# jonathan-innis/karpenter-provider-aws

Hardware: AMD Instinct MI355X
Metric: pods scheduled/sec (Solve, 50k pods × EC2 catalog) (higher is better)
Workload: dtype int64; 1 GPU; config2: 50000 heterogeneous pods (250 classes) x 918 types x 3 AZ x {spot,on-demand}, 2 NodePools; pods=50000, types=918, parallelism=single

## Files before the change

karpenter-provider-aws_amd/csrc/kp_ffd.h:

```cpp
#pragma once
#include <hip/hip_runtime.h>
#include <stdint.h>

#include <type_traits>

#include "kp_bound.h"
#include "kp_device.h"
#include "kp_eval.h"
#include "kp_gosort.h"
#include "kp_layout.h"

namespace KP_WNS {

#ifdef KP_NO_TOPO
#define KP_TOPO_ON 0
#else
#define KP_TOPO_ON 1
#endif

__device__ __forceinline__ bool ports_meet(const KpDev& d, const uint64_t* m, int c) {
    uint64_t x = 0;
    for (int w = 0; w < d.PW; w++)
        x |= __hip_atomic_load(const_cast<uint64_t*>(m) + w, __ATOMIC_RELAXED, __HIP_MEMORY_SCOPE_AGENT) &
             d.cls_ports[(size_t)c * d.PW + w];
// ... 318 lines not shown
        for (uint64_t m = ballot(live); m; m &= m - 1) {
            const int j = __ffsll((unsigned long long)m) - 1;
            const int g = rl32(R.g, j), flags = rl32(R.flags, j), key = rl32(R.key, j);
            if (flags & 8) {
                if (lane == 0) {
                    const int old = atomicAdd(&d.tg_hcnt[(size_t)(-1 - key) * d.HN + d.E + nc], 1);
                    if (old == 0) atomicAdd(&d.tg_pos[g], 1);
                }
                continue;
            }
            const uint64_t wv = rl64(w, j);
            if ((wv >> lane) & 1ull) atomicAdd(&d.tg_cnt[(size_t)g * 64 + lane], 1);
            if (lane == 0 && wv) atomicOr((unsigned long long*)&d.tg_known[g], (unsigned long long)wv);
        }
    }
    if (keep && lane == 0) {
        S.tr_n = nr;
        S.tr_cls = c;
    }
    asm volatile("s_waitcnt vmcnt(0)" ::: "memory");
}

#define KP_CAND_VIRT 0x40000000
#ifndef KP_BOUND_SWEEP
#define KP_BOUND_SWEEP 0
#endif
#ifndef KP_BOUND_IDLE_WAVE
#define KP_BOUND_IDLE_WAVE 1
#endif
#ifndef KP_BOUND_ROW_SKIP
#define KP_BOUND_ROW_SKIP 1
#endif
#ifndef KP_BOUND_TMPL_IDLE
#define KP_BOUND_TMPL_IDLE 1
#endif
template <bool PROF>
static __device__ __attribute__((noinline)) int bound_round(const int64_t* __restrict__ nc_bound,
                                                            const int64_t* __restrict__ nc_req,
                                                            int R, int A,
                                                            FfdShared& S, uint32_t* key, const uint16_t* ord, int buf,
                                                            int cnt, int sdone, int r) {
    static_assert(KP_NWAVES <= 8 && KP_LDS_AXES <= KP_BOUND_STRIDE && KP_BOUND_STRIDE == 8, "lane = 8 candidate + axis");
    const int lane = (int)__lane_id(), ci = lane >> 3, ai = lane & 7;
    const bool v = ci < cnt && ai < A;
    const int nc = ord[S.cand_pos[buf][ci < cnt ? ci : 0]];
    const int64_t b = v ? __hip_atomic_load(const_cast<int64_t*>(&nc_bound[(size_t)nc * KP_BOUND_STRIDE + ai]), __ATOMIC_RELAXED,
                                            __HIP_MEMORY_SCOPE_AGENT) : KP_NO_BOUND;
    const int64_t tot = v ? ld_req(&nc_req[(size_t)nc * R + r]) : 0;
    const uint64_t m = ballot(v && kp_bound_rejects(b, tot, S.pod_req[r]));
    if (!m) return 0;
    uint64_t vm = 0;
    for (int i = 0; i < 8; i++)
        if ((m >> (8 * i)) & 0xFFull) vm |= 1ull << i;
    const int nv = __popcll(vm);
    const int p = lane < cnt ? S.cand_pos[buf][lane] : 0;
    const bool rej = (vm >> lane) & 1ull;
    if (nv == cnt && !sdone) {
        if (rej) key[p] |= 0x80000000u;
        if (lane == 0) {
            S.st[ST_NC_EVALS] += cnt;
            S.st[ST_BOUND_SKIPS] += cnt;
            if (PROF) S.st[ST_BOUND_ALLV]++;
            S.fwd = 1;
        }
        return 1;
    }
    if (rej) S.cand_pos[buf][lane] = p | KP_CAND_VIRT;
    if (PROF && lane == 0) S.st[nv == cnt ? ST_BOUND_ALLV : ST_BOUND_MIXED]++;
    return 0;
}
template <bool TOPO, bool PORTS = false, bool BOUND = false, bool PROF = false>
__device__ inline bool collect_candidates(const KpDev& d, FfdShared& S,
                                          std::conditional_t<PORTS || BOUND, uint32_t*, const uint32_t*> key,
                                          const uint16_t* ord, const uint8_t* stmpl, uint64_t tol, int N, int start, int buf,
                                          int lane, int pc = -1, bool bound = false) {
    int pos = start;
    bool marked = false;
    for (;;) {
        int cnt = 0, next = N;
        const int tp_n = TOPO ? S.tp_n : 0;
        const int L = tp_n ? d.topo_cands : KP_NWAVES;
        while (pos < N) {
            const int p = pos + lane;
            bool c = p < N && !(key[p] >> 31);
            if (c) c = (tol >> stmpl[ord[p]]) & 1ull;
            if (PORTS && pc >= 0) {
                const bool meet = c && ports_meet(d, d.nc_ports + (size_t)ord[p] * d.PW, pc);
                if constexpr (PORTS)
                    if (meet) key[p] |= 0x80000000u;
                marked |= ballot(meet) != 0;
                c = c && !meet;
            }
            if (tp_n && c) c = topo_prefilter_pass(d, S, ord[p]);
            const uint64_t m0 = __ballot(c);
            if (tp_n && m0 && cnt + __popcll(m0) < L) {
                const int rank = cnt + __popcll(m0 & ((1ull << lane) - 1ull));
                if (c) S.cand_pos[buf][rank] = p;
                cnt += __popcll(m0);
                pos += 64;
                if (lane == 0) {
                    S.n_cand[buf] = cnt;
                    S.scan_next[buf] = pos < N ? pos : N;
// ... 98 lines not shown
        if (!pending || base >= TP) break;
#pragma unroll
        for (int ai = 0; ai < KP_LDS_AXES; ai++) t[ai] = ((pending >> ai) & 1u) ? (int)rank[ai * TP + base + lane] : 0xFFFF;
    }
#endif
    tail.hi = (tail.hi & 0x0000FFFFFFFFFFFFull) | ((uint64_t)(unsigned)(first < 0 ? start : first) << 48);
    int64_t mine = KP_NO_BOUND;
#pragma unroll
    for (int ai = 0; ai < KP_LDS_AXES; ai++)
        if (lane == ai) mine = mx[ai];
    if (lane < A)
        __hip_atomic_store(&row[lane], kp_bound_entry(mine, ws.hr[lane] >= 0), __ATOMIC_RELAXED, __HIP_MEMORY_SCOPE_AGENT);
    if (lane == KP_BOUND_STRIDE - 2 || lane == KP_BOUND_STRIDE - 1)
        __hip_atomic_store(&row[lane], (int64_t)(lane == KP_BOUND_STRIDE - 2 ? tail.lo : tail.hi), __ATOMIC_RELAXED,
                           __HIP_MEMORY_SCOPE_AGENT);
}

__device__ __forceinline__ uint64_t limit_filter(const KpDev& d, int j, uint64_t o, int lane) {
    return lane < d.TW ? o & d.tmpl_lmask[(size_t)j * d.TW + lane] : o;
}

__device__ inline void limit_mask_update(const KpDev& d, int j, int lane) {
    uint32_t lm = 0;
    for (int r = 0; r < d.R; r++)
        if (d.limit_set[(size_t)j * d.R + r]) lm |= 1u << r;
    uint64_t mine = ~0ull;
    for (int w = 0; w < d.TW && lm; w++) {
        const int t = w * 64 + lane;
        bool keep = t < d.T;
        for (uint32_t m = lm; m && keep; m &= m - 1) {
            const int r = __ffs(m) - 1;
            keep = d.cap[(size_t)r * d.T + t] <= ld_req(&d.remaining[(size_t)j * d.R + r]);
        }
        const uint64_t nb = ballot(keep);
        if (lane == w) mine = nb;
    }
    if (lane < d.TW) d.tmpl_lmask[(size_t)j * d.TW + lane] = mine;
}

__device__ __forceinline__ long long prof_clock(bool prof) { return prof ? __builtin_amdgcn_s_memtime() : 0; }


__device__ __forceinline__ void commit_reservations(const KpDev& d, int32_t* rcap, const WaveScratch& ws, int nc,
                                                    bool fresh, int* rel_flag, int lane) {
    const int RW = d.ro_ridw;
    if (lane < RW) {
        uint64_t* hp = d.nc_held + (size_t)nc * RW + lane;
        const uint64_t old = fresh ? 0ull : ld_u64(hp), nh = ws.minbits[lane];
        for (uint64_t x = nh & ~old; x; x &= x - 1) rcap[lane * 64 + __ffsll((unsigned long long)x) - 1]--;
        for (uint64_t x = old & ~nh; x; x &= x - 1)
            if (rcap[lane * 64 + __ffsll((unsigned long long)x) - 1]++ == 0) *rel_flag = 1;
        __hip_atomic_store(hp, nh, __ATOMIC_RELAXED, __HIP_MEMORY_SCOPE_AGENT);
    }
    if (lane == 0) __hip_atomic_store(&d.nc_rlive[nc], ws.rlive, __ATOMIC_RELAXED, __HIP_MEMORY_SCOPE_AGENT);
}
__device__ __forceinline__ uint64_t held_word(const KpDev& d, int nc, int lane) {
    return lane < d.ro_ridw ? ld_u64(&d.nc_held[(size_t)nc * d.ro_ridw + lane]) : 0ull;
}

template <bool VOL = false>
// ... 284 lines not shown
        for (int j = 0; j < d.NT; j++)
            if (d.min_keys[(size_t)j * KP_MAX_CLASS_KEYS] >= 0) mmask |= 1ull << j;
        E.min_tmpl_mask = mmask;
    }
    SortSlice sl{skey, sord};
    int my_axis = 0, my_shift = 0;
#pragma unroll
    for (int ai = 0; ai < KP_LDS_AXES; ai++)
        if (lane == ai) {
            my_axis = d.active_axes[ai];
            my_shift = d.qshift[ai];
        }
    const long long pop_bound = (long long)P * 64 + 4096;
    constexpr bool LEAN = !PORTS || TOPO;
    int qw_n = 0, qw_used = 0;
    int vp = 0, vc = 0, vshape = 0, vlast = 0;
    uint64_t vtol = 0;
    int32_t vq[KP_LDS_AXES];
#pragma unroll
    for (int ai = 0; ai < KP_LDS_AXES; ai++) vq[ai] = 0;

    for (;;) {
        const long long c_top = (prof && tid == 0) ? __builtin_amdgcn_s_memtime() : 0;
        if (wave == 0) {
            const long long c_in = prof_clock(prof);
            const int N = S.N;
            int qhead = S.qhead, qcount = S.qcount;
            int seq = S.seq, prev_shape = S.prev_shape, dkind = S.dirty_kind, dpos = S.dirty_pos;
            int sstart = S.scan_start;
            int eager = S.eager;
            int any_rej = S.any_rej;
            const int ep = S.epoch;
            if (PREF && d.relax_next && S.relaxed) {
                vlast = -1;
                __builtin_amdgcn_fence(__ATOMIC_SEQ_CST, "wavefront");
                if (lane == 0) S.relaxed = 0;
            }
            if (RESV && S.rel_flag) {
                for (int i = lane; i < N; i += 64) skey[i] &= KEYMASK;
                any_rej = 0;
                sstart = 0;
                __builtin_amdgcn_fence(__ATOMIC_SEQ_CST, "wavefront");
                if (lane == 0) S.rel_flag = 0;
            }
            int xstart = S.xstart;
            long long nexist = 0;
// ... 566 lines not shown
                            qcount--;
                            popped++;
                            scanned += N;
                            n_inner++;
                            stay = true;
                            break;
                        }
                        t_d = prof_clock(prof);
                        cqinner += t_d - t_e;
                        if (!stay) break;
                        again = false;
                        continue;
                    }
                }
                break;
                }
                if (again) continue;
                t_f = prof_clock(prof);
                ho_fail = t_f - t_d;
                if (prof) {
                    const bool fa = f < N && rl32(wa ? 1 : 0, (f - wb) & 63) != 0;
                    if (lane == 0) S.st[ST_SLOW_WHY + (f >= N ? 0 : A == 0 ? 3 : !fa ? 1 : 2)]++;
                }
                win_flush();
                wb = -1;
                if (lane < R) S.pod_req[lane] = qw_req[off * R + lane];
                if (lane == 0) {
                    S.cur_pod = p;
                    S.cls_fill = S.CC.cls != c;
                    S.topo_pod = 0;
                }
                if (BOUND) asm volatile("s_waitcnt vmcnt(0)" ::: "memory");
                if (BOUND && lane == 0) S.fwd = 0;
                if (collect_candidates<TOPO_ON, PORTS, BOUND, PROF>(d, S, skey, sord, stmpl, ~0ull, N, f, 0, lane,
                                                                          (PORTS && cport) ? c : -1, BOUND))
                    any_rej = 1;
                break;
            }
            win_flush();
            ex_flush();
            const long long t_w = prof_clock(prof);
            if (lane == 0) {
                S.xstart = xstart;
                S.st[ST_EXIST_PLACED] += nexist;
                S.qhead = qhead;
                S.qcount = qcount;
                S.seq = seq;
                S.prev_shape = prev_shape;
                S.dirty_kind = dkind;
                S.dirty_pos = dpos;
                S.scan_start = sstart;
                S.eager = eager;
                S.any_rej = any_rej;
                S.topo_resume = 0;
                S.rej_volatile = 0;
                S.done = done;
// ... 224 lines not shown
                    if (!ok && S.ws[0].memo_ok) {
                        skey[S.cand_pos[b][i]] |= 0x80000000u;
                        S.any_rej = 1;
                    }
                    if (!ok && !S.ws[0].memo_ok) S.rej_volatile = 1;
                    S.st[ST_NC_EVALS]++;
                }
                if (ok) {
                    win = i;
                    break;
                }
            }
            if (win >= 0 || S.scan_done[b]) break;
            if (wave == 0 &&
                collect_candidates<TOPO_ON, PORTS>(d, S, skey, sord, stmpl, S.topo_pod ? d.tol[S.cur_cls] : ~0ull, S.N, S.scan_next[b],
                                                   b ^ 1, lane, (PORTS && (S.CC.flags & CF_PORTS)) ? S.cur_cls : -1) && lane == 0)
                S.any_rej = 1;
            __syncthreads();
            round++;
        }
        int first = 0;
        bool team_won = false;
        if ((KP_TEAM_FIRST_RESV | !RESV) && (KP_TEAM_FIRST_TOPO | !TOPO))
        if (!team && d.team_first && S.n_cand[0] > 0 && !(BOUND && ((S.cand_pos[0][0] & KP_CAND_VIRT) || S.fwd))) {
            const int nc = sord[S.cand_pos[0][0]];
            const int tm = d.nc_tmpl[nc];
            const bool fast0 = !(S.CC.flags & CF_TOPO) && !(RESV && d.resv_on && ld_i32(&d.nc_rlive[nc])) &&
                               (slast[nc] == (uint16_t)S.cur_cls || ((S.CC.flags & CF_NOKEYS) && ((S.CC.tol >> tm) & 1ull)));
            if (!fast0) {
                EvalIn a;
                a.Ahdr = d.nc_hdr + (size_t)nc * K;
                a.Aw = d.nc_words + (size_t)nc * d.DW;
                a.opts = lane < TW ? d.nc_opts[(size_t)nc * TW + lane] : 0;
                a.base_req = d.nc_req + (size_t)nc * R;
                a.pod_req = S.pod_req;
                a.tmpl = tm;
                a.compat = true;
                a.force_off = false;
                a.prof = wave == 0 ? &S.st[ST_EV_REQ] : nullptr;
                a.host = d.E + nc;
                a.held = (RESV && d.resv_on) ? held_word(d, nc, lane) : 0ull;
                TeamBuf* const tb = &S.team[tjoins & 1];
                const bool ok = (TOPO_ON && (S.CC.flags & CF_TOPO_CONS))
                                    ? eval_wave<true, RESV, true, PREF, false, true, PROF>(d, E, S.CC, a, S.ws[wave], lane, tb,
                                                                                     wave, KP_NWAVES, &tjoins)
                                    : eval_wave<false, RESV, true, PREF, false, true, PROF>(d, E, S.CC, a, S.ws[wave], lane,
                                                                                      tb, wave, KP_NWAVES, &tjoins);
                if (wave == 0 && lane == 0) {
                    S.fastp[0][0] = 0;
                    S.acc[0][0] = ok;
                    if (!ok && S.ws[0].memo_ok) {
                        skey[S.cand_pos[0][0]] |= 0x80000000u;
                        S.any_rej = 1;
                    }
                    if (!ok && !S.ws[0].memo_ok) S.rej_volatile = 1;
                    S.st[ST_NC_EVALS]++;
                    if (prof) S.st[ST_SLOW_WHY + 8]++;
                }
                first = 1;
                if (ok) {
                    win = 0;
                    team_won = true;
                }
                __syncthreads();
            }
        }
        for (; !team && !team_won;) {
            const int b = round & 1;
            const int f0 = round == 0 ? first : 0;
            const int ci = wave + f0;
            if (BOUND && ci < S.n_cand[b] && (S.cand_pos[b][ci] & KP_CAND_VIRT)) {
                if (lane == 0) {
                    S.fastp[b][ci] = 0;
                    S.acc[b][ci] = 0;
                    skey[S.cand_pos[b][ci] & ~KP_CAND_VIRT] |= 0x80000000u;
                    S.any_rej = 1;
                    atomicAdd((unsigned long long*)&S.st[ST_BOUND_SKIPS], 1ull);
                }
            } else if (ci < S.n_cand[b]) {
                const int nc = sord[S.cand_pos[b][ci]];
                EvalIn a;
                a.Ahdr = d.nc_hdr + (size_t)nc * K;
                a.Aw = d.nc_words + (size_t)nc * d.DW;
                a.opts = lane < TW ? d.nc_opts[(size_t)nc * TW + lane] : 0;
                a.base_req = d.nc_req + (size_t)nc * R;
// ... 115 lines not shown
            auto commit_tmpl = [&](int jj, int cw) {
                const int n = S.N;
                for (int k = lane; k < K; k += 64) d.nc_hdr[(size_t)n * K + k] = d.cls_hdr[(size_t)(d.C + jj) * K + k];
                for (int i = lane; i < d.DW; i += 64)
                    d.nc_words[(size_t)n * d.DW + i] = d.cls_words[(size_t)(d.C + jj) * d.DW + i];
                asm volatile("s_waitcnt vmcnt(0)" ::: "memory");
                commit_reqs(d, S.CC, S.ws[cw], n, lane);
                if (PREF && d.best_effort) {
                    asm volatile("s_waitcnt vmcnt(0)" ::: "memory");
                    commit_min_relax(d, S.ws[cw], n, lane);
                }
                if (RESV && d.resv_on) commit_reservations(d, sRcap, S.ws[cw], n, true, &S.rel_flag, lane);
                if (TOPO_ON && (S.CC.flags & CF_TOPO))
                    topo_record(d, S.CC, S.ws[cw], d.cls_hdr + (size_t)(d.C + jj) * K,
                                d.cls_words + (size_t)(d.C + jj) * d.DW, d.E + n, jj, true, lane, -1, nullptr,
                                S.born);
                if (lane < TW) d.nc_opts[(size_t)n * TW + lane] = S.ws[cw].opts[lane];
                if (PORTS) nodeclaim_ports_commit(d, n, S.cur_cls, true, jj, lane);
                for (int r = lane; r < R; r += 64)
                    __hip_atomic_store(&d.nc_req[(size_t)n * R + r], d.daemon[(size_t)jj * R + r] + S.pod_req[r],
                                       __ATOMIC_RELAXED, __HIP_MEMORY_SCOPE_AGENT);
                if (lane < A && n < NQ) shr[lane * NQ + n] = S.ws[cw].hr[lane];
                if (BOUND && !KP_BOUND_TMPL_IDLE) bound_row_store<PROF>(d.self, E.alloc, S.ws[cw], n, 0, S.st);
                for (int r = 0; r < R; r++) {
                    if (!d.limit_set[(size_t)jj * R + r]) continue;
                    int64_t mx = INT64_MIN;
                    for (int w2 = 0; w2 < TW; w2++) {
                        const uint64_t ow = S.ws[cw].opts[w2];
                        if ((ow >> lane) & 1ull) {
                            const int64_t cp = d.cap[(size_t)r * T + w2 * 64 + lane];
                            mx = cp > mx ? cp : mx;
                        }
                    }
                    mx = wave_max64(mx);
                    if (lane == 0) d.remaining[(size_t)jj * R + r] -= mx;
                }
                asm volatile("s_waitcnt vmcnt(0)" ::: "memory");
                limit_mask_update(d, jj, lane);
                if (lane == 0) {
                    slast[n] = (uint16_t)S.cur_cls;
                    stmpl[n] = (uint8_t)jj;
                    d.nc_tmpl[n] = jj;
                    sord[n] = (uint16_t)n;
                    skey[n] = 1;
                    S.N = n + 1;
                    S.dirty_kind = 2;
                    S.dirty_pos = n;
                    d.pod_result[pod] = n;
                    d.pod_order[pod] = S.seq++;
                }
                asm volatile("s_waitcnt vmcnt(0)" ::: "memory");
            };
            int twin = -1;
            if (KP_TEAM_TMPL && (!RESV || KP_TEAM_TMPL_RESV) && !TOPO && d.team_first) {
                const int n_new = BOUND ? S.N : 0;
                for (int j = 0; j < d.NT; j++) {
                    uint64_t o = (lane < TW && d.tmpl_ok[j]) ? d.tmpl_opts[(size_t)j * TW + lane] : 0;
                    o = limit_filter(d, j, o, lane);
                    if (PORTS && (S.CC.flags & CF_PORTS) && ports_meet(d, d.tmpl_ports + (size_t)j * d.PW, S.cur_cls)) o = 0;
                    if (!ballot(o != 0)) continue;
                    EvalIn a;
// ... 93 lines not shown
                        const int n = S.N;
                        for (int k = lane; k < K; k += 64) d.nc_hdr[(size_t)n * K + k] = d.cls_hdr[(size_t)(d.C + jj) * K + k];
                        for (int i = lane; i < d.DW; i += 64)
                            d.nc_words[(size_t)n * d.DW + i] = d.cls_words[(size_t)(d.C + jj) * d.DW + i];
                        asm volatile("s_waitcnt vmcnt(0)" ::: "memory");
                        commit_reqs(d, S.CC, S.ws[wave], n, lane);
                        if (PREF && d.best_effort) {
                            asm volatile("s_waitcnt vmcnt(0)" ::: "memory");
                            commit_min_relax(d, S.ws[wave], n, lane);
                        }
                        if (RESV && d.resv_on) commit_reservations(d, sRcap, S.ws[wave], n, true, &S.rel_flag, lane);
                        if (TOPO_ON && (S.CC.flags & CF_TOPO))
                            topo_record(d, S.CC, S.ws[wave], d.cls_hdr + (size_t)(d.C + jj) * K,
                                        d.cls_words + (size_t)(d.C + jj) * d.DW, d.E + n, jj, true, lane, -1, nullptr,
                                        S.born);
                        if (lane < TW) d.nc_opts[(size_t)n * TW + lane] = S.ws[wave].opts[lane];
                        if (PORTS) nodeclaim_ports_commit(d, n, S.cur_cls, true, jj, lane);
                        for (int r = lane; r < R; r += 64)
                            __hip_atomic_store(&d.nc_req[(size_t)n * R + r], d.daemon[(size_t)jj * R + r] + S.pod_req[r],
                                               __ATOMIC_RELAXED, __HIP_MEMORY_SCOPE_AGENT);
                        if (lane < A && n < NQ) shr[lane * NQ + n] = S.ws[wave].hr[lane];
                        if (BOUND)
                            bound_row_store<PROF>(d.self, E.alloc, S.ws[wave], n, KP_BOUND_TMPL_IDLE ? d.tmpl_bstep[jj] : 0, S.st);
                        for (int r = 0; r < R; r++) {
                            if (!d.limit_set[(size_t)jj * R + r]) continue;
                            int64_t mx = INT64_MIN;
                            for (int w2 = 0; w2 < TW; w2++) {
                                const uint64_t ow = S.ws[wave].opts[w2];
                                if ((ow >> lane) & 1ull) {
                                    const int64_t cp = d.cap[(size_t)r * T + w2 * 64 + lane];
                                    mx = cp > mx ? cp : mx;
                                }
                            }
                            mx = wave_max64(mx);
                            if (lane == 0) d.remaining[(size_t)jj * R + r] -= mx;
                        }
                        asm volatile("s_waitcnt vmcnt(0)" ::: "memory");
                        limit_mask_update(d, jj, lane);
                        if (lane == 0) {
                            slast[n] = (uint16_t)S.cur_cls;
                            stmpl[n] = (uint8_t)jj;
                            d.nc_tmpl[n] = jj;
                            sord[n] = (uint16_t)n;
                            skey[n] = 1;
                            S.N = n + 1;
                            S.dirty_kind = 2;
                            S.dirty_pos = n;
                            d.pod_result[pod] = n;
                            d.pod_order[pod] = S.seq++;
                        }
                        asm volatile("s_waitcnt vmcnt(0)" ::: "memory");
                    }
                    break;
                }
                __syncthreads();
            }
            if (tid == 0) {
                if (prof) S.st[ST_CYC_TMPL] += __builtin_amdgcn_s_memtime() - c_t;
                if (twin < 0) {
                    const int tail = (S.qhead + S.qcount) % P;
                    d.qbuf[tail] = pod;
// ... 83 lines not shown
```

karpenter-provider-aws_amd/csrc/kp_host.cpp:

```cpp
#include <hip/hip_runtime.h>

#include <arpa/inet.h>

#include <algorithm>
#include <array>
#include <atomic>
#include <cfloat>
#include <chrono>
#include <cstdint>
#include <cstdio>
#include <cstring>
#include <map>
#include <set>
#include <memory>
#include <string>
#include <condition_variable>
#include <functional>
#include <mutex>
#include <thread>
#include <unordered_map>
#include <vector>

#include "../../include/kpsim.h"
#include "kp_gosort_host.h"
#include "kp_cons.h"
#include "kp_launch.h"
#include "kp_layout.h"

#include "kp_bound.h"
#include "kp_host.h"

namespace {

using clk = std::chrono::steady_clock;
double ns_since(clk::time_point t0) { return std::chrono::duration<double, std::nano>(clk::now() - t0).count(); }

bool go_atoi(const char* s, int64_t& out) {
    size_t n = strlen(s), i = 0;
    bool neg = false;
    if (n == 0) return false;
    if (s[0] == '+' || s[0] == '-') {
        neg = s[0] == '-';
        i = 1;
    }
    if (i >= n) return false;
    unsigned __int128 v = 0;
    for (; i < n; i++) {
        if (s[i] < '0' || s[i] > '9') return false;
        v = v * 10 + (unsigned)(s[i] - '0');
        if (v > (unsigned __int128)1 << 63) return false;
    }
    if (!neg && v > (unsigned __int128)INT64_MAX) return false;
// ... 314 lines not shown
    DBuf<int64_t> d_alloc, d_cap;
    DBuf<double> d_slot_price;
    DBuf<int32_t> d_slot_zone, d_slot_ct, d_slot_zoneid;
    DBuf<uint32_t> d_name_rank;
    bool prepared = false, executed = false;
    Dicts sol;
    KpDev dev{};
    int P = 0, C = 0, NT = 0, K = 0, DW = 0;
    std::vector<int> tmpl_np;
    std::vector<int64_t> h_remaining;
    DBuf<uint32_t> d_kflags, d_cls_flags;
    DBuf<uint64_t> d_tol;
    DBuf<uint64_t> d_cls_ports, d_tmpl_ports, d_ex_ports0, d_ex_ports, d_nc_ports;
    DBuf<int32_t> d_shape_vs, d_vs_cnt, d_ex_vlim, d_ex_vcnt0, d_ex_vcnt;
    DBuf<uint64_t> d_vs_mask, d_drv_mask, d_ex_vmask0, d_ex_vmask;
    DBuf<uint8_t> d_ex_vover;
    DBuf<ReqHdr> d_ex_hdr0, d_ex_hdr;
    DBuf<uint64_t> d_ex_words0, d_ex_words, d_ex_tol, d_XT;
    DBuf<int64_t> d_ex_avail, d_ex_req, d_ex_head;
    DBuf<uint8_t> d_ex_static;
    DBuf<int32_t> d_cls_xkoff, d_cls_xkeys;
    DBuf<int32_t> d_kcat, d_kmulti, d_woff, d_nw, d_nval, d_vbase, d_cls_koff, d_cls_keys, d_cls_wsoff, d_min_keys;
    DBuf<uint8_t> d_val_isint, d_limit_set;
    DBuf<int64_t> d_val_int, d_daemon, d_remaining, d_pod_req, d_sort_fields, d_nc_req, d_stats;
    DBuf<uint64_t> d_tmpl_lmask;
    DBuf<ReqHdr> d_cls_hdr, d_nc_hdr, d_empty_hdr;
    DBuf<uint64_t> d_cls_words, d_V, d_tmpl_rows, d_tmpl_opts, d_nc_words, d_nc_opts, d_empty_words, d_keys_a, d_keys_b;
    DBuf<int32_t> d_tmpl_ok, d_pod_cls, d_pod_shape, d_perm_a, d_perm_b, d_nc_tmpl, d_qbuf, d_last_len, d_pod_result,
        d_pod_order, d_nc_count, d_nc_npods, d_nc_slice_pos, d_nc_nopts, d_nc_valid, d_nc_types, d_nc_ntypes, d_err;
    DBuf<char> d_sort_temp;
    size_t sort_temp_bytes = 0;
    double ns_prep = 0, ns_exec = 0, ns_fin = 0;
    hipEvent_t ev[6] = {};
    double kernel_ms[5] = {};
    int64_t cycles[49] = {};
    bool any_min_values = false;
    int max_min_values = 0;
    bool min_multi = false;
    std::vector<uint8_t> cons_mutcls;
    DBuf<int32_t> d_retry, d_rank, d_cand_i, d_cand_off, d_cand_pods, d_pending, d_ring, d_ring_last, d_next, d_pnode;
    DBuf<double> d_cand_price;
    DBuf<int64_t> d_cand_cap, d_delta, d_alloc_act, d_cons_stats, d_cmax0, d_alloc_stage;
    std::vector<int32_t> h_uid_p;
    std::vector<uint64_t> h_uid_k;
    std::vector<int32_t> h_shape_tab;
    int nc_cap_once = 0;
    int last_plan_nc = 0;
    bool nc_overflow = false;
    DBuf<uint64_t> d_pend_bits, d_pbits;
    DBuf<uint64_t> d_ubits;
    DBuf<int32_t> d_rcand, d_ulen;
    DBuf<int2> d_ulist;
    DBuf<uint64_t> d_init;
    DBuf<kp_probe_result> d_probe_out;
    DBuf<int32_t> d_rec_i;
    DBuf<int64_t> d_prof_probe;
    DBuf<ReqHdr> d_rec_hdr;
    DBuf<uint64_t> d_rec_words;
// ... 1462 lines not shown
    } while (0)
struct SolveEnc {
    std::vector<std::map<int, HReq>> creq, cstrict, treq;
    std::vector<std::vector<std::map<int, HReq>>> cfilt;
    std::vector<int> npo;
    TopoHost th;
    int E = 0, EW = 0, NT = 0, CT = 0, K = 0, DW = 0, NCcap = 0, M = 0, hostname_key = -1;
    std::vector<std::vector<std::pair<int, int>>> exlab;
    std::map<int, int> host_node;
    std::vector<uint32_t> kflags;
    std::vector<int32_t> kcat, kmulti, woff, nw, nval, vbase;
    std::vector<uint8_t> isint;
    std::vector<int64_t> ival;
    std::vector<ReqHdr> chdr;
    std::vector<uint64_t> cwords;
    std::vector<uint32_t> cflags;
    std::vector<int32_t> koff, ckeys, cwsoff, min_keys, xkoff, xkeys;
    std::vector<uint8_t> ckneu, hblock;
    std::vector<int2> frow;
    bool mayfix = false;
    std::vector<uint64_t> tol, rows, exw, extol;
    std::vector<int64_t> daemon, remaining, exav, exrq;
    std::vector<uint8_t> limit_set;
    std::vector<ReqHdr> exhdr;
    std::vector<int32_t> shape_next;
    int PW = 0, port_bits = 0;
    std::vector<uint64_t> cports, tports, xports;
    int VD = 0, VW = 0, vol_bits = 0;
    std::vector<int32_t> pod_vs;
    std::vector<int32_t> shape_vs;
    std::vector<int32_t> vs_cnt, ex_vlim, ex_vcnt;
    std::vector<uint64_t> vs_mask, drv_mask, ex_vmask;
    std::vector<uint8_t> ex_vover;
    std::vector<int32_t> vol_drivers;
};

static kp_status solve_expand(kp_ctx* ctx, const kp_solve_input* in, SolveEnc& se) {
    ctx->any_min_values = false;
    ctx->max_min_values = 0;
    ctx->min_multi = false;
    if (in->min_values_policy != KP_MIN_VALUES_STRICT && in->min_values_policy != KP_MIN_VALUES_BEST_EFFORT)
        return fail(ctx, KP_E_INVALID, "unknown MIN_VALUES_POLICY");
    ctx->best_effort = in->min_values_policy == KP_MIN_VALUES_BEST_EFFORT;
    if (in->n_classes < 0 || (in->n_classes > 0 && !in->classes)) return fail(ctx, KP_E_INVALID, "pod classes");
    for (int i = 0; i < in->pods.n_pods; i++)
        if (in->pods.class_id[i] < 0 || in->pods.class_id[i] >= in->n_classes)
// ... 286 lines not shown
        for (int i = 0; i < C; i++) {
            bool all = true;
            for (int q = 0; q < np.n_taints && all; q++)
                all = tolerates(np.taints[q], in->classes[i].tolerations, in->classes[i].n_tolerations);
            if (all) se.tol[i] |= 1ull << j;
        }
        for (int r = 0; r < R; r++) {
            if (np.daemon_overhead) se.daemon[(size_t)j * R + r] = np.daemon_overhead[r];
            if (np.limit_set && np.limit_set[r]) {
                se.limit_set[(size_t)j * R + r] = 1;
                se.remaining[(size_t)j * R + r] = np.limit_remaining[r];
            }
        }
        if (np.n_types < 0) {
            for (int t = 0; t < T; t++) se.rows[(size_t)j * TW + t / 64] |= 1ull << (t % 64);
        } else {
            for (int q = 0; q < np.n_types; q++) {
                const int t = np.type_index[q];
                if (t < 0 || t >= T) return fail(ctx, KP_E_INVALID, "nodepool type_index out of range");
                se.rows[(size_t)j * TW + t / 64] |= 1ull << (t % 64);
            }
        }
    }
    ctx->h_x_tol = se.tol;
    ctx->h_x_hblock = se.hblock;
    ctx->x_host_key = se.hostname_key;
    for (int i = 0; i < C; i++)
        if (se.hblock[i]) se.tol[i] = 0;
    return KP_OK;
}

static kp_status solve_existing_digests(kp_ctx* ctx, const kp_solve_input* in, SolveEnc& se) {
    const int R = ctx->R, C = in->n_classes, E = se.E, K = se.K, DW = se.DW;
    const int EW = se.EW = (E + 63) / 64;
    se.exhdr.resize((size_t)std::max(E, 1) * K);
    memset(se.exhdr.data(), 0, se.exhdr.size() * sizeof(ReqHdr));
    se.exw.assign((size_t)std::max(E, 1) * DW, 0), se.extol.assign((size_t)std::max(C, 1) * std::max(EW, 1), 0);
    se.exav.assign((size_t)std::max(E, 1) * R, 0), se.exrq.assign((size_t)std::max(E, 1) * R, 0);
    for (int j = 0; j < E; j++) {
        const kp_existing_node& en = in->existing[j];
        for (auto& kv : se.exlab[j]) {
            ReqHdr& h = se.exhdr[(size_t)j * K + kv.first];
            h.flags = RF_DEF;
            se.exw[(size_t)j * DW + se.woff[kv.first] + kv.second / 64] |= 1ull << (kv.second % 64);
        }
        for (int r = 0; r < R; r++) {
// ... 471 lines not shown
    HIPCHK(c->d_tmpl_ok.ensure(std::max(NT, 1)));
    HIPCHK(c->d_tol.upload(se.tol, s));
    if (se.PW > 0) {
        HIPCHK(c->d_cls_ports.upload(se.cports, s));
        HIPCHK(c->d_tmpl_ports.upload(se.tports, s));
        HIPCHK(c->d_ex_ports0.upload(se.xports, s));
        HIPCHK(c->d_ex_ports.ensure(se.xports.size()));
    }
    if (se.VD > 0) {
        if (se.shape_vs.empty()) se.shape_vs.push_back(0);
        HIPCHK(c->d_shape_vs.upload(se.shape_vs, s));
        HIPCHK(c->d_vs_cnt.upload(se.vs_cnt, s));
        HIPCHK(c->d_vs_mask.upload(se.vs_mask, s));
        HIPCHK(c->d_drv_mask.upload(se.drv_mask, s));
        HIPCHK(c->d_ex_vlim.upload(se.ex_vlim, s));
        HIPCHK(c->d_ex_vcnt0.upload(se.ex_vcnt, s));
        HIPCHK(c->d_ex_vcnt.ensure(se.ex_vcnt.size()));
        HIPCHK(c->d_ex_vmask0.upload(se.ex_vmask, s));
        HIPCHK(c->d_ex_vmask.ensure(se.ex_vmask.size()));
        HIPCHK(c->d_ex_vover.upload(se.ex_vover, s));
    }
    HIPCHK(c->d_daemon.upload(se.daemon, s));
    HIPCHK(c->d_limit_set.upload(se.limit_set, s));
    HIPCHK(c->d_remaining.upload(se.remaining, s));
    c->h_remaining = se.remaining;
    HIPCHK(c->d_min_keys.upload(se.min_keys, s));
    if (se.xkeys.empty()) se.xkeys.push_back(0);
    HIPCHK(c->d_cls_xkoff.upload(se.xkoff, s));
    HIPCHK(c->d_cls_xkeys.upload(se.xkeys, s));
    HIPCHK(c->d_ex_hdr0.upload(se.exhdr, s));
    HIPCHK(c->d_ex_words0.upload(se.exw, s));
    HIPCHK(c->d_ex_hdr.ensure(se.exhdr.size()));
    HIPCHK(c->d_ex_words.ensure(se.exw.size()));
    HIPCHK(c->d_ex_avail.upload(se.exav, s));
    HIPCHK(c->d_ex_req.upload(se.exrq, s));
    HIPCHK(c->d_ex_head.ensure((size_t)KP_MAX_R * std::max(E, 1)));
    HIPCHK(c->d_ex_static.ensure(std::max(E, 1)));
    HIPCHK(c->d_ex_tol.upload(se.extol, s));
    HIPCHK(c->d_XT.ensure(se.extol.size()));
    HIPCHK(c->d_pod_cls.upload(c->p_pcls.p, P, s));
    HIPCHK(c->d_pod_shape.upload(c->p_pshape.p, P, s));
    if (!se.shape_next.empty()) {
        HIPCHK(c->d_pod_cls0.upload(c->p_pcls.p, P, s));
        HIPCHK(c->d_pod_shape0.upload(c->p_pshape.p, P, s));
        HIPCHK(c->d_relax_next.upload(c->pref.relax_next, s));
        HIPCHK(c->d_shape_next.upload(se.shape_next, s));
// ... 399 lines not shown
    const int E = se.E, EW = se.EW, NT = se.NT, K = se.K, DW = se.DW, NCcap = se.NCcap, M = se.M;
    hipStream_t s = c->stream;
    KpDev& d = c->dev;
    d.T = T;
    d.TW = TW;
    d.R = R;
    d.K = K;
    d.n_slots = c->n_slots;
    d.n_multi = c->n_multi;
    DEV(type_val); DEV(multi_mask);
    d.multi16 = c->multi16_ok ? c->d_multi16.p : nullptr;
    DEV(dne_mask); DEV(alloc); DEV(cap); DEV(avail_zc); DEV(slot_price); DEV(slot_zone); DEV(slot_ct); DEV(slot_zoneid);
    DEV(name_rank); DEV(nonneg); DEV(kflags); DEV(kcat); DEV(kmulti); DEV(woff); DEV(nw); DEV(nval); DEV(vbase);
    DEV(val_isint); DEV(val_int);
    d.DW = DW;
    d.key_zone = c->key_zone;
    d.key_ct = c->key_ct;
    d.key_zoneid = c->key_zoneid;
    d.key_resvid = c->key_resvid;
    d.key_resvtype = c->key_resvtype;
    d.C = C;
    d.NT = NT;
    DEV(cls_koff); DEV(cls_keys); DEV(cls_wsoff); DEV(cls_hdr); DEV(cls_words); DEV(cls_flags); DEV(V); DEV(tmpl_rows);
    DEV(tmpl_opts); DEV(tmpl_ok); DEV(tol); DEV(daemon); DEV(limit_set); DEV(remaining);
    d.PW = se.PW;
    if (se.PW > 0) {
        DEV(cls_ports); DEV(tmpl_ports); DEV(ex_ports0); DEV(ex_ports); DEV(nc_ports);
    }
    d.VD = se.VD;
    d.VW = se.VW;
    if (se.VD > 0) {
        DEV(shape_vs); DEV(vs_cnt); DEV(vs_mask); DEV(drv_mask); DEV(ex_vlim); DEV(ex_vcnt0); DEV(ex_vcnt); DEV(ex_vmask0);
        DEV(ex_vmask); DEV(ex_vover);
    }
    HIPCHK(c->d_tmpl_lmask.ensure((size_t)std::max(1, d.NT) * std::max(1, d.TW)));
    DEV(tmpl_lmask); DEV(min_keys);
    d.E = E;
    d.EW = EW;
    DEV(ex_hdr0); DEV(ex_words0); DEV(ex_hdr); DEV(ex_words); DEV(ex_avail); DEV(ex_req); DEV(ex_head); DEV(ex_static);
    DEV(XT); DEV(ex_tol); DEV(cls_xkoff); DEV(cls_xkeys);
    d.ex_mayfix = se.mayfix ? 1 : 0;
    d.P = P;
    DEV(pod_cls); DEV(pod_shape);
    const bool relax = !c->pref.relax_next.empty();
    d.relax_next = relax ? c->d_relax_next.p : nullptr;
    d.shape_next = relax ? c->d_shape_next.p : nullptr;
    d.pod_cls0 = relax ? c->d_pod_cls0.p : nullptr;
// ... 310 lines not shown
    so.pods_popped = st[ST_POPPED];
    so.nodeclaim_evals = st[ST_NC_EVALS];
    so.nodeclaim_candidates_scanned = st[ST_NC_SCANNED];
    so.template_evals = st[ST_TMPL_EVALS];
    so.existing_evals = st[ST_EXIST_PLACED];
    so.sorts_fast = st[ST_SORT_FAST];
    so.sorts_full = st[ST_SORT_FULL];
    for (int i = 0; i < 6; i++) c->cycles[i] = st[ST_CYC_POP + i];
    for (int i = 0; i < 6; i++) c->cycles[6 + i] = st[ST_EV_REQ + i];
    for (int i = 0; i < 7; i++) c->cycles[12 + i] = st[ST_QUICK + i];
    for (int i = 0; i < 11; i++) c->cycles[19 + i] = st[ST_N_NOINV + i];
    for (int i = 0; i < 3; i++) c->cycles[30 + i] = st[ST_TOPO_QUICK + i];
    for (int i = 0; i < 4; i++) c->cycles[33 + i] = st[ST_REJ_REQ + i];
    for (int i = 0; i < 3; i++) c->cycles[37 + i] = st[ST_HANDOFF + i];
    c->cycles[40] = st[ST_HANDOFF_WB];
    c->cycles[41] = st[ST_N_INNER];
    c->cycles[42] = st[ST_CYC_QINNER];
    c->cycles[43] = st[ST_N_MULTI];
    c->cycles[44] = st[ST_BOUND_SKIPS];
    c->cycles[45] = st[ST_BOUND_ALLV];
    c->cycles[46] = st[ST_BOUND_MIXED];
    c->cycles[47] = st[ST_SORT_FULL_WIDE];
    c->cycles[48] = st[ST_CYC_SORT_FULL_WIDE];
    if (getenv("KPSIM_PROFILE") && st[ST_SLOW_WHY] + st[ST_SLOW_WHY + 1] + st[ST_SLOW_WHY + 2] + st[ST_SLOW_WHY + 3])
        fprintf(stderr, "[kpsim] slow-path pods: no candidate %lld, class not absorbed %lld, witness short %lld, no witness table %lld; "
                "no-op merge quick accepts %lld; placed by the first candidate %lld, a later one %lld, the templates %lld; "
                "block-evaluated first candidates %lld; cycles: commit + templates %lld, class cache fills %lld\n",
                (long long)st[ST_SLOW_WHY], (long long)st[ST_SLOW_WHY + 1], (long long)st[ST_SLOW_WHY + 2],
                (long long)st[ST_SLOW_WHY + 3], (long long)st[ST_SLOW_WHY + 4], (long long)st[ST_SLOW_WHY + 5],
                (long long)st[ST_SLOW_WHY + 6], (long long)st[ST_SLOW_WHY + 7], (long long)st[ST_SLOW_WHY + 8],
                (long long)st[ST_SLOW_WHY + 9], (long long)st[ST_SLOW_WHY + 10]);
    if (getenv("KPSIM_PROFILE") && st[ST_TQ_WHY] + st[ST_TQ_WHY + 1] + st[ST_TQ_WHY + 2] + st[ST_TQ_WHY + 3] + st[ST_TQ_WHY + 4])
        fprintf(stderr, "[kpsim] topology pods past the prefilter: no survivor %lld, not QREC %lld, no quick row %lld, class not "
                        "absorbed %lld, quick row %lld (witness fits %lld, merge no-op %lld); NQ %d of %d NodeClaims\n",
                (long long)st[ST_TQ_WHY], (long long)st[ST_TQ_WHY + 1], (long long)st[ST_TQ_WHY + 2], (long long)st[ST_TQ_WHY + 3],
                (long long)st[ST_TQ_WHY + 4], (long long)st[ST_TQ_WHY + 5], (long long)st[ST_TQ_WHY + 6], c->dev.lds_nq, N);
    if (getenv("KPSIM_PROFILE") && st[ST_SEG])
        fprintf(stderr, "[kpsim] solve loop segments (cycles): fast loop + slow-path entry %lld, topology section %lld "
                        "(topology quick accepts: %lld iterations, %lld cycles from the slow-path entry), class cache %lld, "
                        "evaluations %lld, commit / templates / slice move %lld\n",
                (long long)st[ST_SEG], (long long)st[ST_SEG + 1], (long long)st[ST_TQ_ITERS], (long long)st[ST_TQ_CYC],
                (long long)st[ST_SEG + 2], (long long)st[ST_SEG + 3], (long long)st[ST_SEG + 4]);
    so.ns_host_prep = c->ns_prep;
    so.ns_device_solve = c->ns_exec;
    if (N > out->cap_nodeclaims || n_ids > out->cap_type_ids) return fail(ctx, KP_E_BUFFER, "output buffers too small");
    int off = 0;
// ... 5 lines not shown
        out->nodeclaim_type_offset[i] = off;
        for (int q = 0; q < ntypes[i]; q++) out->type_ids[off++] = types[(size_t)i * M + q];
    }
    out->nodeclaim_type_offset[N] = off;
    for (int p = 0; p < P; p++) {
        int r = pres[p];
        int o = pord[p];
        if (r >= 0 && !valid[r]) {
            r = KP_POD_UNSCHEDULABLE;
            o = -1;
        }
        out->pod_result[p] = r;
        if (out->pod_order) out->pod_order[p] = o;
    }
    so.ns_device_finalize = ns_since(t0);
    so.ns_total = c->ns_prep + c->ns_exec + so.ns_device_finalize;
    return KP_OK;
}

extern "C" kp_status kp_last_kernel_times(kp_ctx* ctx, double* ms, int32_t n) {
    if (!ctx || !ms) return KP_E_INVALID;
    if (!ctx->executed) return fail(ctx, KP_E_STATE, "no execute yet");
    for (int i = 0; i < n && i < 5; i++) ms[i] = ctx->kernel_ms[i];
    for (int i = 5; i < n && i < 54; i++) ms[i] = (double)ctx->cycles[i - 5];
    return KP_OK;
}

extern "C" kp_status kp_solve(kp_ctx* ctx, const kp_solve_input* in, kp_solve_output* out) {
    for (int attempt = 0;; attempt++) {
        kp_status st = kp_solve_prepare(ctx, in);
        if (st != KP_OK) return st;
        st = kp_solve_execute(ctx);
        if (st != KP_OK) return st;
        st = kp_solve_fetch(ctx, out);
        const int want = std::min(KP_MAX_NC, std::max(in->pods.n_pods, 1));
        if (st == KP_E_UNSUPPORTED && ctx->nc_overflow && attempt == 0 && ctx->last_plan_nc < want) continue;
        ctx->nc_cap_once = 0;
        return st;
    }
}

static std::string reqs_text(const kp_ctx* ctx, const ReqHdr* h, const uint64_t* w);

extern "C" kp_status kp_result_nodeclaim_requirements(kp_ctx* ctx, int32_t nc, char* buf, int64_t cap, int64_t* needed) {
    if (!ctx) return KP_E_INVALID;
    if (!ctx->executed) return fail(ctx, KP_E_STATE, "no solve result");
    if (nc < 0 || nc >= ctx->last_N) return fail(ctx, KP_E_INVALID, "nodeclaim index");
// ... 2462 lines not shown
```

karpenter-provider-aws_amd/csrc/kp_layout.h:

```cpp
#pragma once
#include <stdint.h>

#ifndef KP_MAX_TYPES
#define KP_MAX_TYPES 2048
#endif
#define KP_TW_MAX (KP_MAX_TYPES / 64)
#define KP_DNE_TW 16
#define KP_MAX_NC 65535
#define KP_NC_FIRST 4096
#define KP_MAX_KEYS 96
#define KP_MAX_CLASS_KEYS 32
#define KP_MAX_SLOTS 64
#define KP_MAX_NP 63
#define KP_MAX_R 16
#ifndef KP_NWAVES
#define KP_NWAVES 8
#endif
#ifndef KP_NWAVES_TOPO
#define KP_NWAVES_TOPO 4
#endif
#define KP_WNS_CAT2(n) kp_w##n
#define KP_WNS_CAT(n) KP_WNS_CAT2(n)
#define KP_WNS KP_WNS_CAT(KP_NWAVES)
#define KP_LDS_AXES 6
// ... 99 lines not shown
    const int32_t* nval;
    const int32_t* vbase;
    const uint8_t* val_isint;
    const int64_t* val_int;
    int32_t DW;
    int32_t key_zone, key_ct, key_zoneid, key_resvid, key_resvtype;

    int32_t C;
    int32_t NT;
    const int32_t* cls_koff;
    const int32_t* cls_keys;
    const int32_t* cls_wsoff;
    const ReqHdr* cls_hdr;
    const uint64_t* cls_words;
    const uint32_t* cls_flags;
    uint64_t* V;

    const uint64_t* tmpl_rows;
    uint64_t* tmpl_opts;
    int32_t* tmpl_ok;
    const uint64_t* tol;
    const int64_t* daemon;
    const uint8_t* limit_set;
    int64_t* remaining;
    uint64_t* tmpl_lmask;
    const int32_t* min_keys;

    int32_t P;
    int32_t* pod_cls;
    int32_t* pod_shape;
    const int32_t* relax_next;
    const int32_t* shape_next;
    const int32_t* pod_cls0;
    const int32_t* pod_shape0;
    int32_t* last_ep;
    int32_t best_effort;
    const int64_t* pod_req;
    const int32_t* queue0;
    int32_t active_axes[KP_MAX_R];
    int32_t n_active;

    int32_t NCcap;
    ReqHdr* nc_hdr;
    uint64_t* nc_words;
    uint64_t* nc_opts;
    int64_t* nc_req;
// ... 113 lines not shown
    const uint64_t* drv_mask;
    const int32_t* ex_vlim;
    const int32_t* ex_vcnt0;
    int32_t* ex_vcnt;
    const uint64_t* ex_vmask0;
    uint64_t* ex_vmask;
    const uint8_t* ex_vover;
};

enum {
    ST_POPPED = 0, ST_NC_EVALS, ST_NC_SCANNED, ST_TMPL_EVALS, ST_EXIST_EVALS, ST_SORT_FAST, ST_SORT_FULL,
    ST_BOUND_MIXED, ST_CYC_POP, ST_CYC_SORT, ST_CYC_SCAN, ST_CYC_TMPL, ST_CYC_COMMIT, ST_CYC_SORT_FULL,
    ST_N_INNER = 14, ST_CYC_QINNER, ST_N_MULTI = 22,
    ST_BOUND_SKIPS = 23, ST_BOUND_ALLV = 31,
    ST_BOUND_ROWS = 46,
    ST_SORT_FULL_WIDE = 75, ST_CYC_SORT_FULL_WIDE = 76,
    ST_EV_REQ = 16, ST_EV_MASK, ST_EV_OFF, ST_EV_TYPES, ST_EV_MIN, ST_EV_CALLS,
    ST_QUICK = 24, ST_SLOW, ST_WITNESS_MISS, ST_CYC_QPOP, ST_CYC_QSCAN, ST_CYC_QCHECK, ST_CYC_QCOMMIT,
    ST_N_NOINV = 32, ST_N_WINMOVE, ST_N_LDSSORT, ST_N_PIVOT, ST_N_WINLOAD, ST_N_FLUSH, ST_N_SHAPE, ST_EXIST_PLACED = 44,
    ST_TOPO_QUICK = 45, ST_CYC_TSETUP, ST_CYC_TSCAN,
    ST_REJ_REQ = 48, ST_REJ_TOPO, ST_REJ_TYPES, ST_REJ_MIN,
    ST_TQ_WHY = 52, ST_SLOW_WHY = 59,
    ST_SEG = 70, ST_TQ_ITERS = 75, ST_TQ_CYC = 76,
    ST_HANDOFF = 77, ST_HANDOFF_WB = 43, ST_COUNT = 80
};
static_assert(ST_BOUND_ROWS == ST_CYC_TSETUP, "ST_BOUND_ROWS shares the topology setup slot");
static_assert(ST_SORT_FULL_WIDE == ST_TQ_ITERS && ST_CYC_SORT_FULL_WIDE == ST_TQ_CYC, "the full-sort split shares the topology quick-accept slots");
```

Measured before the change: 732,600 pods/s.

## Hand off a fitting first candidate alone and precompute template limit-axis masks

```diff
diff --git a/karpenter-provider-aws_amd/csrc/kp_ffd.h b/karpenter-provider-aws_amd/csrc/kp_ffd.h
--- a/karpenter-provider-aws_amd/csrc/kp_ffd.h
+++ b/karpenter-provider-aws_amd/csrc/kp_ffd.h
@@ -364,6 +364,8 @@
 }
 
 #define KP_CAND_VIRT 0x40000000
+#define KP_FWD_PASSED 1
+#define KP_FWD_FIRST_ALONE 2
 #ifndef KP_BOUND_SWEEP
 #define KP_BOUND_SWEEP 0
 #endif
@@ -375,6 +377,12 @@
 #endif
 #ifndef KP_BOUND_TMPL_IDLE
 #define KP_BOUND_TMPL_IDLE 1
+#endif
+#ifndef KP_HO_FIRST
+#define KP_HO_FIRST 1
+#endif
+#ifndef KP_TMPL_LIMMASK
+#define KP_TMPL_LIMMASK 1
 #endif
 template <bool PROF>
 static __device__ __attribute__((noinline)) int bound_round(const int64_t* __restrict__ nc_bound,
@@ -403,7 +411,7 @@
             S.st[ST_NC_EVALS] += cnt;
             S.st[ST_BOUND_SKIPS] += cnt;
             if (PROF) S.st[ST_BOUND_ALLV]++;
-            S.fwd = 1;
+            S.fwd = KP_FWD_PASSED;
         }
         return 1;
     }
@@ -411,15 +419,17 @@
     if (PROF && lane == 0) S.st[nv == cnt ? ST_BOUND_ALLV : ST_BOUND_MIXED]++;
     return 0;
 }
-template <bool TOPO, bool PORTS = false, bool BOUND = false, bool PROF = false>
+template <bool TOPO, bool PORTS = false, bool BOUND = false, bool PROF = false, int TAKEN = 0>
 __device__ inline bool collect_candidates(const KpDev& d, FfdShared& S,
                                           std::conditional_t<PORTS || BOUND, uint32_t*, const uint32_t*> key,
                                           const uint16_t* ord, const uint8_t* stmpl, uint64_t tol, int N, int start, int buf,
                                           int lane, int pc = -1, bool bound = false) {
     int pos = start;
     bool marked = false;
+    int taken = TAKEN;
     for (;;) {
-        int cnt = 0, next = N;
+        int cnt = taken, next = N;
+        taken = 0;
         const int tp_n = TOPO ? S.tp_n : 0;
         const int L = tp_n ? d.topo_cands : KP_NWAVES;
         while (pos < N) {
@@ -564,8 +574,12 @@
 
 __device__ inline void limit_mask_update(const KpDev& d, int j, int lane) {
     uint32_t lm = 0;
+#if KP_TMPL_LIMMASK
+    lm = d.tmpl_limax[j];
+#else
     for (int r = 0; r < d.R; r++)
         if (d.limit_set[(size_t)j * d.R + r]) lm |= 1u << r;
+#endif
     uint64_t mine = ~0ull;
     for (int w = 0; w < d.TW && lm; w++) {
         const int t = w * 64 + lane;
@@ -578,6 +592,32 @@
         if (lane == w) mine = nb;
     }
     if (lane < d.TW) d.tmpl_lmask[(size_t)j * d.TW + lane] = mine;
+}
+
+__device__ inline void limits_commit(const KpDev& d, int jj, const uint64_t* opts, int lane) {
+    const int R = d.R, T = d.T, TW = d.TW;
+#if KP_TMPL_LIMMASK
+    const uint32_t lm = (uint32_t)__builtin_amdgcn_readfirstlane((int)d.tmpl_limax[jj]);
+    if (!lm) return;
+    for (uint32_t m = lm; m; m &= m - 1) {
+        const int r = __ffs(m) - 1;
+#else
+    for (int r = 0; r < R; r++) {
+        if (!d.limit_set[(size_t)jj * R + r]) continue;
+#endif
+        int64_t mx = INT64_MIN;
+        for (int w2 = 0; w2 < TW; w2++) {
+            const uint64_t ow = opts[w2];
+            if ((ow >> lane) & 1ull) {
+                const int64_t cp = d.cap[(size_t)r * T + w2 * 64 + lane];
+                mx = cp > mx ? cp : mx;
+            }
+        }
+        mx = wave_max64(mx);
+        if (lane == 0) d.remaining[(size_t)jj * R + r] -= mx;
+    }
+    asm volatile("s_waitcnt vmcnt(0)" ::: "memory");
+    limit_mask_update(d, jj, lane);
 }
 
 __device__ __forceinline__ long long prof_clock(bool prof) { return prof ? __builtin_amdgcn_s_memtime() : 0; }
@@ -908,6 +948,7 @@
 
     for (;;) {
         const long long c_top = (prof && tid == 0) ? __builtin_amdgcn_s_memtime() : 0;
+        bool ho_elig = false;
         if (wave == 0) {
             const long long c_in = prof_clock(prof);
             const int N = S.N;
@@ -1520,6 +1561,20 @@
                     const bool fa = f < N && rl32(wa ? 1 : 0, (f - wb) & 63) != 0;
                     if (lane == 0) S.st[ST_SLOW_WHY + (f >= N ? 0 : A == 0 ? 3 : !fa ? 1 : 2)]++;
                 }
+                bool ho_first = false;
+                if constexpr (BOUND && (KP_HO_FIRST || PROF)) {
+                    if (f < N && wb >= 0 && f >= wb && f < wb + 64 && d.team_first && !(tl >> 63)) {
+                        bool wfit = A > 0;
+#pragma unroll
+                        for (int ai = 0; ai < KP_LDS_AXES; ai++)
+                            if (ai < A) wfit &= pq[ai] <= wh[ai];
+                        const int fl = f - wb;
+                        const int tm = (int)((uint32_t)rl32((int)wm, fl) >> 16);
+                        ho_first = ((ballot(wfit && !wa) >> fl) & 1ull) && ((tl >> tm) & 1ull);
+                    }
+                    if (PROF && ho_first && lane == 0) S.st[ST_HO_FIRST]++;
+                    ho_elig = ho_first;
+                }
                 win_flush();
                 wb = -1;
                 if (lane < R) S.pod_req[lane] = qw_req[off * R + lane];
@@ -1528,8 +1583,15 @@
                     S.cls_fill = S.CC.cls != c;
                     S.topo_pod = 0;
                 }
+                if (BOUND && lane == 0) S.fwd = (KP_HO_FIRST && ho_first) ? KP_FWD_FIRST_ALONE : 0;
+                if (BOUND && KP_HO_FIRST && ho_first) {
+                    if (lane == 0) {
+                        S.cand_pos[0][0] = f;
+                        S.n_cand[0] = 1;
+                    }
+                    break;
+                }
                 if (BOUND) asm volatile("s_waitcnt vmcnt(0)" ::: "memory");
-                if (BOUND && lane == 0) S.fwd = 0;
                 if (collect_candidates<TOPO_ON, PORTS, BOUND, PROF>(d, S, skey, sord, stmpl, ~0ull, N, f, 0, lane,
                                                                           (PORTS && cport) ? c : -1, BOUND))
                     any_rej = 1;
@@ -1800,7 +1862,7 @@
         int first = 0;
         bool team_won = false;
         if ((KP_TEAM_FIRST_RESV | !RESV) && (KP_TEAM_FIRST_TOPO | !TOPO))
-        if (!team && d.team_first && S.n_cand[0] > 0 && !(BOUND && ((S.cand_pos[0][0] & KP_CAND_VIRT) || S.fwd))) {
+        if (!team && d.team_first && S.n_cand[0] > 0 && !(BOUND && ((S.cand_pos[0][0] & KP_CAND_VIRT) || S.fwd == KP_FWD_PASSED))) {
             const int nc = sord[S.cand_pos[0][0]];
             const int tm = d.nc_tmpl[nc];
             const bool fast0 = !(S.CC.flags & CF_TOPO) && !(RESV && d.resv_on && ld_i32(&d.nc_rlive[nc])) &&
@@ -1834,11 +1896,20 @@
                     if (!ok && !S.ws[0].memo_ok) S.rej_volatile = 1;
                     S.st[ST_NC_EVALS]++;
                     if (prof) S.st[ST_SLOW_WHY + 8]++;
+                    if (BOUND && PROF && !ok && ho_elig) S.st[ST_HO_FIRST_REJ]++;
                 }
                 first = 1;
                 if (ok) {
                     win = 0;
                     team_won = true;
+                }
+                if constexpr (BOUND && KP_HO_FIRST) {
+                    if (!ok && wave == 0 && S.fwd == KP_FWD_FIRST_ALONE) {
+                        const int p0 = S.cand_pos[0][0];
+                        if (collect_candidates<TOPO_ON, PORTS, BOUND, PROF, 1>(d, S, skey, sord, stmpl, ~0ull, S.N, p0 + 1, 0,
+                                                                                lane, -1, true) && lane == 0)
+                            S.any_rej = 1;
+                    }
                 }
                 __syncthreads();
             }
@@ -2000,21 +2071,7 @@
                                        __ATOMIC_RELAXED, __HIP_MEMORY_SCOPE_AGENT);
                 if (lane < A && n < NQ) shr[lane * NQ + n] = S.ws[cw].hr[lane];
                 if (BOUND && !KP_BOUND_TMPL_IDLE) bound_row_store<PROF>(d.self, E.alloc, S.ws[cw], n, 0, S.st);
-                for (int r = 0; r < R; r++) {
-                    if (!d.limit_set[(size_t)jj * R + r]) continue;
-                    int64_t mx = INT64_MIN;
-                    for (int w2 = 0; w2 < TW; w2++) {
-                        const uint64_t ow = S.ws[cw].opts[w2];
-                        if ((ow >> lane) & 1ull) {
-                            const int64_t cp = d.cap[(size_t)r * T + w2 * 64 + lane];
-                            mx = cp > mx ? cp : mx;
-                        }
-                    }
-                    mx = wave_max64(mx);
-                    if (lane == 0) d.remaining[(size_t)jj * R + r] -= mx;
-                }
-                asm volatile("s_waitcnt vmcnt(0)" ::: "memory");
-                limit_mask_update(d, jj, lane);
+                limits_commit(d, jj, S.ws[cw].opts, lane);
                 if (lane == 0) {
                     slast[n] = (uint16_t)S.cur_cls;
                     stmpl[n] = (uint8_t)jj;
@@ -2154,21 +2211,7 @@
                         if (lane < A && n < NQ) shr[lane * NQ + n] = S.ws[wave].hr[lane];
                         if (BOUND)
                             bound_row_store<PROF>(d.self, E.alloc, S.ws[wave], n, KP_BOUND_TMPL_IDLE ? d.tmpl_bstep[jj] : 0, S.st);
-                        for (int r = 0; r < R; r++) {
-                            if (!d.limit_set[(size_t)jj * R + r]) continue;
-                            int64_t mx = INT64_MIN;
-                            for (int w2 = 0; w2 < TW; w2++) {
-                                const uint64_t ow = S.ws[wave].opts[w2];
-                                if ((ow >> lane) & 1ull) {
-                                    const int64_t cp = d.cap[(size_t)r * T + w2 * 64 + lane];
-                                    mx = cp > mx ? cp : mx;
-                                }
-                            }
-                            mx = wave_max64(mx);
-                            if (lane == 0) d.remaining[(size_t)jj * R + r] -= mx;
-                        }
-                        asm volatile("s_waitcnt vmcnt(0)" ::: "memory");
-                        limit_mask_update(d, jj, lane);
+                        limits_commit(d, jj, S.ws[wave].opts, lane);
                         if (lane == 0) {
                             slast[n] = (uint16_t)S.cur_cls;
                             stmpl[n] = (uint8_t)jj;
diff --git a/karpenter-provider-aws_amd/csrc/kp_host.cpp b/karpenter-provider-aws_amd/csrc/kp_host.cpp
--- a/karpenter-provider-aws_amd/csrc/kp_host.cpp
+++ b/karpenter-provider-aws_amd/csrc/kp_host.cpp
@@ -28,6 +28,7 @@
 #include "kp_layout.h"
 
 #include "kp_bound.h"
+#include "kp_limits.h"
 #include "kp_host.h"
 
 namespace {
@@ -388,6 +389,7 @@
     DBuf<int32_t> d_cls_xkoff, d_cls_xkeys;
     DBuf<int32_t> d_kcat, d_kmulti, d_woff, d_nw, d_nval, d_vbase, d_cls_koff, d_cls_keys, d_cls_wsoff, d_min_keys;
     DBuf<uint8_t> d_val_isint, d_limit_set;
+    DBuf<uint32_t> d_tmpl_limax;
     DBuf<int64_t> d_val_int, d_daemon, d_remaining, d_pod_req, d_sort_fields, d_nc_req, d_stats;
     DBuf<uint64_t> d_tmpl_lmask;
     DBuf<ReqHdr> d_cls_hdr, d_nc_hdr, d_empty_hdr;
@@ -399,7 +401,7 @@
     double ns_prep = 0, ns_exec = 0, ns_fin = 0;
     hipEvent_t ev[6] = {};
     double kernel_ms[5] = {};
-    int64_t cycles[49] = {};
+    int64_t cycles[51] = {};
     bool any_min_values = false;
     int max_min_values = 0;
     bool min_multi = false;
@@ -1908,6 +1910,7 @@
     std::vector<uint64_t> tol, rows, exw, extol;
     std::vector<int64_t> daemon, remaining, exav, exrq;
     std::vector<uint8_t> limit_set;
+    std::vector<uint32_t> limax;
     std::vector<ReqHdr> exhdr;
     std::vector<int32_t> shape_next;
     int PW = 0, port_bits = 0;
@@ -2240,6 +2243,9 @@
             }
         }
     }
+    static_assert(KP_MAX_R <= KP_LIMAX_BITS, "a template's limited axes fit one word");
+    se.limax.assign(std::max(NT, 1), 0);
+    kp_limit_axes_all(se.limit_set.data(), NT, R, se.limax.data());
     ctx->h_x_tol = se.tol;
     ctx->h_x_hblock = se.hblock;
     ctx->x_host_key = se.hostname_key;
@@ -2757,6 +2763,7 @@
     }
     HIPCHK(c->d_daemon.upload(se.daemon, s));
     HIPCHK(c->d_limit_set.upload(se.limit_set, s));
+    HIPCHK(c->d_tmpl_limax.upload(se.limax, s));
     HIPCHK(c->d_remaining.upload(se.remaining, s));
     c->h_remaining = se.remaining;
     HIPCHK(c->d_min_keys.upload(se.min_keys, s));
@@ -3202,7 +3209,7 @@
     d.C = C;
     d.NT = NT;
     DEV(cls_koff); DEV(cls_keys); DEV(cls_wsoff); DEV(cls_hdr); DEV(cls_words); DEV(cls_flags); DEV(V); DEV(tmpl_rows);
-    DEV(tmpl_opts); DEV(tmpl_ok); DEV(tol); DEV(daemon); DEV(limit_set); DEV(remaining);
+    DEV(tmpl_opts); DEV(tmpl_ok); DEV(tol); DEV(daemon); DEV(limit_set); DEV(tmpl_limax); DEV(remaining);
     d.PW = se.PW;
     if (se.PW > 0) {
         DEV(cls_ports); DEV(tmpl_ports); DEV(ex_ports0); DEV(ex_ports); DEV(nc_ports);
@@ -3559,6 +3566,8 @@
     c->cycles[46] = st[ST_BOUND_MIXED];
     c->cycles[47] = st[ST_SORT_FULL_WIDE];
     c->cycles[48] = st[ST_CYC_SORT_FULL_WIDE];
+    c->cycles[49] = c->tg_G > 0 ? 0 : st[ST_HO_FIRST];
+    c->cycles[50] = c->tg_G > 0 ? 0 : st[ST_HO_FIRST_REJ];
     if (getenv("KPSIM_PROFILE") && st[ST_SLOW_WHY] + st[ST_SLOW_WHY + 1] + st[ST_SLOW_WHY + 2] + st[ST_SLOW_WHY + 3])
         fprintf(stderr, "[kpsim] slow-path pods: no candidate %lld, class not absorbed %lld, witness short %lld, no witness table %lld; "
                 "no-op merge quick accepts %lld; placed by the first candidate %lld, a later one %lld, the templates %lld; "
@@ -3610,7 +3619,7 @@
     if (!ctx || !ms) return KP_E_INVALID;
     if (!ctx->executed) return fail(ctx, KP_E_STATE, "no execute yet");
     for (int i = 0; i < n && i < 5; i++) ms[i] = ctx->kernel_ms[i];
-    for (int i = 5; i < n && i < 54; i++) ms[i] = (double)ctx->cycles[i - 5];
+    for (int i = 5; i < n && i < 56; i++) ms[i] = (double)ctx->cycles[i - 5];
     return KP_OK;
 }
 
diff --git a/karpenter-provider-aws_amd/csrc/kp_layout.h b/karpenter-provider-aws_amd/csrc/kp_layout.h
--- a/karpenter-provider-aws_amd/csrc/kp_layout.h
+++ b/karpenter-provider-aws_amd/csrc/kp_layout.h
@@ -145,6 +145,7 @@
     const uint64_t* tol;
     const int64_t* daemon;
     const uint8_t* limit_set;
+    const uint32_t* tmpl_limax;
     int64_t* remaining;
     uint64_t* tmpl_lmask;
     const int32_t* min_keys;
@@ -304,7 +305,10 @@
     ST_REJ_REQ = 48, ST_REJ_TOPO, ST_REJ_TYPES, ST_REJ_MIN,
     ST_TQ_WHY = 52, ST_SLOW_WHY = 59,
     ST_SEG = 70, ST_TQ_ITERS = 75, ST_TQ_CYC = 76,
-    ST_HANDOFF = 77, ST_HANDOFF_WB = 43, ST_COUNT = 80
-};
+    ST_HANDOFF = 77, ST_HANDOFF_WB = 43,
+    ST_HO_FIRST = 52, ST_HO_FIRST_REJ = 53,
+    ST_COUNT = 80
+};
+static_assert(ST_HO_FIRST == ST_TQ_WHY && ST_HO_FIRST_REJ == ST_TQ_WHY + 1, "the first-candidate hand-off counters share topology slots");
 static_assert(ST_BOUND_ROWS == ST_CYC_TSETUP, "ST_BOUND_ROWS shares the topology setup slot");
 static_assert(ST_SORT_FULL_WIDE == ST_TQ_ITERS && ST_CYC_SORT_FULL_WIDE == ST_TQ_CYC, "the full-sort split shares the topology quick-accept slots");
diff --git a/karpenter-provider-aws_amd/csrc/kp_limits.h b/karpenter-provider-aws_amd/csrc/kp_limits.h
--- /dev/null
+++ b/karpenter-provider-aws_amd/csrc/kp_limits.h
@@ -0,0 +1,15 @@
+#pragma once
+#include <stdint.h>
+
+#define KP_LIMAX_BITS 32
+
+inline uint32_t kp_limit_axes(const uint8_t* row, int R) {
+    uint32_t m = 0;
+    for (int r = 0; r < R && r < KP_LIMAX_BITS; r++)
+        if (row[r]) m |= 1u << r;
+    return m;
+}
+
+inline void kp_limit_axes_all(const uint8_t* limit_set, int NT, int R, uint32_t* out) {
+    for (int j = 0; j < NT; j++) out[j] = kp_limit_axes(limit_set + (size_t)j * R, R);
+}
```

Result: no change. 737,600 pods/s (median of 6 runs) (+0.7%).
